# sj-shoff/ImageProcessor

Hardware: AMD Instinct MI355X
Metric: images/sec (resize+thumb+watermark) on 1080p batch at 1/2/4/8 MI355X (higher is better)
Workload: dtype f32+f64

## Files before the change

imageprocessor_amd/csrc/ipx_device.h:

```cpp
#pragma once

#include "ipx_internal.h"

namespace ipx {
namespace {

constexpr uint32_t kM = 0xffffu;

template <int C>
__device__ __forceinline__ double widen(uint32_t px)
{
    constexpr uint32_t sel = 0x0c0c0000u | (uint32_t)C | ((uint32_t)C << 8);
    return (double)__builtin_amdgcn_perm(0u, px, sel);
}

template <int C>
__device__ __forceinline__ uint32_t lerp_channel(uint32_t p00, uint32_t p10, uint32_t p01,
                                                 uint32_t p11, double xw0, double xw1, double yw0,
                                                 double yw1)
{
    const double s00 = widen<C>(p00), s10 = widen<C>(p10);
    const double s01 = widen<C>(p01), s11 = widen<C>(p11);
    const double top = xw0 * s00 + xw1 * s10;
    const double bot = xw0 * s01 + xw1 * s11;
// ... 1 lines not shown
    return (uint32_t)v;
}

__device__ __forceinline__ uint32_t pack_src(uint32_t pr, uint32_t pg, uint32_t pb, uint32_t pa)
{
    return (pr >> 8) | (pg & 0xff00u) | ((pb & 0xff00u) << 8) | ((pa & 0xff00u) << 16);
}

__device__ __forceinline__ uint32_t blend_over(uint32_t d, uint32_t pr, uint32_t pg, uint32_t pb,
                                               uint32_t pa)
{
    const uint32_t pa1 = (kM - pa) * 0x101u;
    const uint32_t r = (((d & 0xffu) * pa1 / kM + pr) >> 8) & 0xffu;
    const uint32_t g = ((((d >> 8) & 0xffu) * pa1 / kM + pg) >> 8) & 0xffu;
    const uint32_t b = ((((d >> 16) & 0xffu) * pa1 / kM + pb) >> 8) & 0xffu;
    const uint32_t a = (((d >> 24) * pa1 / kM + pa) >> 8) & 0xffu;
    return r | (g << 8) | (b << 16) | (a << 24);
}

__device__ __forceinline__ uint32_t glyph_over(uint32_t d, uint32_t mask8, uint32_t sr, uint32_t sg,
                                               uint32_t sb, uint32_t sa)
{
    const uint32_t ma = mask8 | (mask8 << 8);
    const uint32_t a = (kM - (sa * ma / kM)) * 0x101u;
    const uint32_t r = (((d & 0xffu) * a + sr * ma) / kM >> 8) & 0xffu;
    const uint32_t g = ((((d >> 8) & 0xffu) * a + sg * ma) / kM >> 8) & 0xffu;
    const uint32_t b = ((((d >> 16) & 0xffu) * a + sb * ma) / kM >> 8) & 0xffu;
    const uint32_t al = (((d >> 24) * a + sa * ma) / kM >> 8) & 0xffu;
    return r | (g << 8) | (b << 16) | (al << 24);
}

__device__ __forceinline__ uint32_t glyph_run(uint32_t d, int x, int y, const DevGlyph *__restrict__ gl,
                                              int n, uint32_t sr, uint32_t sg, uint32_t sb,
                                              uint32_t sa)
{
    for (int g = 0; g < n; g++) {
        const DevGlyph G = gl[g];
        if (x >= G.x0 && x < G.x1 && y >= G.y0 && y < G.y1) {
            const uint32_t m = G.mask[(size_t)(y - G.y0) * G.mstride + (x - G.x0)];
            if (m) d = glyph_over(d, m, sr, sg, sb, sa);
        }
    }
    return d;
}

template <int PX, int ROWS, int YSTEP>
__device__ __forceinline__ void glyph_walk(const DevGlyph *tab, int n, int x, int ybase, Rect bbox, uint32_t (&d)[ROWS][PX], uint32_t sr,
                                           uint32_t sg, uint32_t sb, uint32_t sa)
{
    static_assert(PX >= 1 && PX <= 4, "a row's mask bytes travel in one dword");
    for (int g = 0; g < n; g += 4) {
        uint32_t m[4][ROWS];
        bool any = false;
#pragma unroll
        for (int j = 0; j < 4; j++) {
            const DevGlyph G = tab[min(g + j, n - 1)];
#pragma unroll
            for (int r = 0; r < ROWS; r++) {
                const int y = ybase + YSTEP * r;
                const bool iny = g + j < n && y >= G.y0 && y < G.y1 && y < bbox.y1;
                uint32_t mm = 0u;
#pragma unroll
                for (int k = 0; k < PX; k++) {
                    const bool in = iny && x + k >= G.x0 && x + k < G.x1;
                    mm |= (in ? (uint32_t)G.mask[(size_t)(y - G.y0) * G.mstride + (x + k - G.x0)] : 0u) << (8 * k);
                    any |= in;
                }
                m[j][r] = mm;
            }
        }
        if (!__any(any)) continue;
#pragma unroll
        for (int j = 0; j < 4; j++)
#pragma unroll
            for (int r = 0; r < ROWS; r++)
#pragma unroll
                for (int k = 0; k < PX; k++) {
                    const uint32_t mk = (m[j][r] >> (8 * k)) & 0xffu;
                    if (mk) d[r][k] = glyph_over(d[r][k], mk, sr, sg, sb, sa);
                }
    }
}

}
}
```

imageprocessor_amd/csrc/ipx_internal.h:

```cpp
#pragma once

#include <hip/hip_runtime.h>

#include <cstdarg>
#include <cstdint>
#include <cstdio>
#include <map>
#include <mutex>

#include "../../include/ipx.h"

namespace ipx {

void set_error(const char *fmt, ...) __attribute__((format(printf, 1, 2)));
void clear_error();
int status_of_exception() noexcept;
#define IPX_CATCH_STATUS catch (...) { return ipx::status_of_exception(); }

#define IPX_HIP(call)                                                                        \
    do {                                                                                     \
        hipError_t e_ = (call);                                                              \
        if (e_ != hipSuccess) {                                                              \
            ipx::set_error("%s failed: %s (%s:%d)", #call, hipGetErrorString(e_), __FILE__,  \
                           __LINE__);                                                        \
            return IPX_ERR_HIP;                                                              \
        }                                                                                    \
    } while (0)

constexpr long long kMaxFrameSpan = 0x7fff0000LL;
constexpr int kMaxFrameSide = 65535;
inline bool frame_span_ok(long long w, long long h, long long stride, int bpp)
{
    if (w > kMaxFrameSide || h > kMaxFrameSide) return false;
    return w <= 0 || h <= 0 || (h - 1) * stride + w * bpp <= kMaxFrameSpan;
}

struct Rect {
    int x0, y0, x1, y1;
    int dx() const { return x1 - x0; }
    int dy() const { return y1 - y0; }
    bool empty() const { return x0 >= x1 || y0 >= y1; }
    Rect shifted(int ox, int oy) const { return Rect{x0 + ox, y0 + oy, x1 + ox, y1 + oy}; }
    Rect intersect(const Rect &s) const;
};
inline Rect to_rect(const ipx_rect &r) { return Rect{r.x0, r.y0, r.x1, r.y1}; }

bool draw_clip(Rect &r, int dw, int dh, bool has_src, int sw, int sh, int &spx, int &spy,
               bool has_mask, int mw, int mh, int &mpx, int &mpy);

enum SrcType { kSrcRGBA, kSrcNRGBA, kSrcGray, kSrcPaletted, kSrcYCbCr, kSrcNRGBA64, kSrcRGBA64, kSrcGray16, kSrcCMYK, kSrcTypes };
inline int src_bpp(int type) { static const int b[kSrcTypes] = {4, 4, 1, 1, 1, 8, 8, 2, 4}; return b[type]; }
inline int src_of_deep(int k) { return k >= IPX_DEEP_NRGBA64 && k <= IPX_DEEP_CMYK ? kSrcNRGBA64 + k : -1; }
inline int src_of_png(int k)
{
    static const int t[] = {kSrcGray, kSrcNRGBA, kSrcRGBA, kSrcPaletted, kSrcGray16, kSrcRGBA64, kSrcNRGBA64};
    return k >= 0 && k < 7 ? t[k] : -1;
}
inline int src_of_job(int k)
{
    static const int t[] = {kSrcRGBA, -1, kSrcNRGBA, kSrcGray, kSrcNRGBA64, kSrcRGBA64, kSrcGray16, kSrcCMYK};
    return k >= 0 && k < 8 ? t[k] : -1;
}
inline void chroma_size(int ratio, int w, int h, int *cw, int *ch)
{
    *cw = ratio == IPX_YCBCR_422 || ratio == IPX_YCBCR_420 ? (w + 1) / 2 : w;
    *ch = ratio == IPX_YCBCR_420 || ratio == IPX_YCBCR_440 ? (h + 1) / 2 : h;
}

enum { IPX_SRC_RGBA = 0, IPX_SRC_NRGBA = 1, IPX_SRC_YCBCR = 2,
       IPX_SRC_TAP64 = 3  };
hipError_t launch_opaque_scan(const uint8_t *src, int sw, int sh, int sstride, int *flag,
                              hipStream_t s);
hipError_t launch_opaque_scan_tap64(const uint8_t *src, int sw, int sh, int sstride, int *flag, hipStream_t s);
hipError_t launch_draw(uint8_t *dst, int dstride, const uint8_t *src, int sstride, int w, int h,
                       int op, hipStream_t s);
hipError_t launch_draw_nrgba(uint8_t *dst, int dstride, const uint8_t *src, int sstride, int w, int h, int op,
                             hipStream_t s, int nframes = 1, size_t dst_fs = 0, size_t src_fs = 0);
hipError_t launch_deep_expand(uint8_t *dst, size_t dst_fs, const uint8_t *src, int sstride, size_t src_fs, int kind, int w, int h, int nframes, hipStream_t s);
hipError_t launch_draw_tap64(uint8_t *dst, int dstride, const uint8_t *src, int sstride, int w, int h, int op, hipStream_t s,
                             int nframes = 1, size_t dst_fs = 0, size_t src_fs = 0);
hipError_t launch_draw_ycbcr(uint8_t *dst, int dstride, const uint8_t *y, int ystride, const uint8_t *cb,
                             const uint8_t *cr, int cstride, int ratio, int spx, int spy, int w, int h, hipStream_t s,
                             int nframes = 1, size_t dst_fs = 0, size_t y_fs = 0, size_t c_fs = 0);

struct DevGlyph {
    const uint8_t *mask;
    int mstride;
    int x0, y0, x1, y1;
};
constexpr int kMaxGlyphs = 256;
hipError_t launch_stream_copy(void *dst, const void *src, size_t bytes, hipStream_t s);
hipError_t launch_composite(uint8_t *dst, int dstride, size_t frame_stride, int nframes,
                            const DevGlyph *glyphs_dev, int n, Rect bbox, uint32_t sr, uint32_t sg,
                            uint32_t sb, uint32_t sa, hipStream_t s);

hipError_t launch_gray_expand(uint8_t *dst, size_t dst_fs, const uint8_t *src, int sstride, size_t src_fs, int w, int h, int n, hipStream_t s);
hipError_t launch_palette_expand(uint8_t *dst, size_t dst_fs, const uint8_t *src, int sstride, size_t src_fs, const uint8_t *palettes, int w,
                                 int h, int n, hipStream_t s);

struct KernelLaunchCache {
    std::mutex mu;
    size_t lds_max = 0;
    std::map<size_t, int> resident;
    bool said = false;
    hipError_t prepare(const void *fn, int threads, size_t lds, int *res)
    {
        std::lock_guard<std::mutex> lk(mu);
        if (lds > lds_max) {
            hipError_t e = hipFuncSetAttribute(fn, hipFuncAttributeMaxDynamicSharedMemorySize, (int)lds);
            if (e != hipSuccess) return e;
            lds_max = lds;
        }
        if (res) {
            auto it = resident.find(lds);
            if (it == resident.end()) {
                int n = 0;
                hipError_t e = hipOccupancyMaxActiveBlocksPerMultiprocessor(&n, fn, threads, lds);
                if (e != hipSuccess) return e;
                it = resident.emplace(lds, n > 1 ? n : 1).first;
            }
            *res = it->second;
        }
        return hipSuccess;
    }
    bool first_report() { std::lock_guard<std::mutex> lk(mu); const bool f = !said; said = true; return f; }
};


struct JpegTables {
    uint8_t quant[2][64];
    uint16_t div8[2][64];
    uint32_t recip[2][64];
};
void jpeg_tables(int quality, JpegTables *t);
struct JpegArgs {
    const uint8_t *src; size_t frame_stride; int stride, w, h;
    int aligned16;
    int16_t *coefs; int mcus_per_frame;
    const uint32_t *huff;
    uint32_t *aclen;
    int16_t *dcq;
    uint32_t recip[2][64];
    uint16_t div8[2][64];
};
hipError_t launch_jpeg_fdct(const JpegArgs &a, int n, hipStream_t s);


struct JpegDecInfo {
    int w, h, h0, v0, ratio, ri, ncomp;
    int host_scans;
    int progressive;
    uint8_t td[3], ta[3];
    size_t scan_off, scan_len;
};
struct JpegDecTables {
    uint16_t lut[4][256];
    int32_t maxcode[4][18];
    int32_t valoff[4][18];
    uint8_t vals[4][256];
    uint16_t qnat[3][64];
    uint32_t bound[4][8];
};
struct JpegDecImage {
    unsigned long long scan_off; uint32_t scan_len, img, first_mcu, n_mcu;
    uint8_t td[3], ta[3], valid, pad;
    uint8_t strict_end, rsv[3];
    unsigned long long uoff;
    uint32_t tab_img, rsv2;
};
struct JpegDecArgs {
    const uint8_t *blob; const JpegDecImage *img; const JpegDecTables *tab;
    int16_t *coefs; int *status;
    int16_t *dcs;
// ... 67 lines not shown
```

imageprocessor_amd/csrc/ipx_ks.h:

```cpp
#pragma once

#include <vector>

#include "ipx_internal.h"

namespace ipx {

struct KsAxis {
    int dw = 0, sw = 0;
    int ntap = 0;
    std::vector<int32_t> lo, cnt;
    std::vector<double> w;
    std::vector<double> itw, itwffff;
    std::vector<double> ones;
};
bool ks_build_axis(int dw, int sw, KsAxis *out);

struct KsAxisDev {
    const int32_t *lo, *cnt;
    const double *w, *itw, *itwffff, *ones;
    int ntap;
};
size_t ks_axis_bytes(const KsAxis &a);
void ks_axis_pack(const KsAxis &a, uint8_t *h, const uint8_t *d, KsAxisDev *out);

enum {
    IPX_SRC_RGBA_CROP = 8,
    IPX_SRC_NRGBA_CROP = 9,
    IPX_SRC_YCBCR_CROP = 10,
    IPX_SRC_TAP64_CROP = 11
};
inline int ks_crop_kind(int kind)
{
    return kind == IPX_SRC_NRGBA ? IPX_SRC_NRGBA_CROP : kind == IPX_SRC_YCBCR ? IPX_SRC_YCBCR_CROP : kind == IPX_SRC_TAP64 ? IPX_SRC_TAP64_CROP
                                                                                                                           : IPX_SRC_RGBA_CROP;
}

struct KsGenArgs {
    uint8_t *dst; int dstride; size_t dst_fs;
    int dr_x0, dr_y0;
    int adr_x0, adr_y0, adr_x1, adr_y1;
    int sr_x0, sr_y0;
    KsAxisDev ax, ay;
    int op;
    const int *opaque_flag;
    int kind;
    const uint8_t *src; int sstride; size_t src_fs;
    const uint8_t *cb, *cr; int cstride, ratio; size_t c_fs;
    int nframes;
    int src_w;
};
hipError_t launch_ks_generic(const KsGenArgs &a, hipStream_t s);

}

namespace ipx {

struct KsStrip { int c0, c1, t0, tw; };
struct KsSeg { int ys, r0, r1; };
template <int NACC> struct KsRowT { double w[NACC], itw[NACC], ones[NACC]; int32_t emit[NACC]; float wf[NACC]; };
static_assert(sizeof(KsRowT<2>) == 64 && sizeof(KsRowT<4>) == 128, "row entries are copied dword-wise");

struct KsFusedOut {
    uint8_t *out; size_t frame_stride; int ostride, obytes;
    int dw, dh, sr_x0, sr_y0;
    int kind;
    int mode, aone;
    int pk;
    int ntap;
    int waves, cpl;
    int wcols;
    const double *wx;
    const float *wxf;
    int split, ntapf;
    float feps;
    const double *itwf;
    const int32_t *xlo;
    const int32_t *colb;
    const void *rows;
    const int32_t *rowoff;
};
struct KsFusedArgs {
    const uint8_t *src; size_t src_fs; int sstride, sw, sh;
    int src_kind;
    int taps_le_alpha;
    const uint8_t *cb, *cr; int cstride, ratio; size_t c_fs;
    uint8_t *wm; size_t wm_fs; int wm_stride;
    int nframes, nstrips, nseg, nthreads, pitch, dbuf;
    const KsStrip *strips; const KsSeg *segs;
    int nout; KsFusedOut o[2];
    int lds_w[2], lds_rows, lds_open;
    int open_per_wave;
    uint8_t wave_role[16];
    unsigned long long *stamps;
    int *redo;
    uint2 *fix; int *fix_count; int fix_cap[2], fix_stride;
};
struct KsText { const DevGlyph *gl; int n; Rect bbox; uint32_t sr, sg, sb, sa; };
struct KsFix { uint2 *list = nullptr; int *count = nullptr; int cap[2] = {0, 0}; KsAxisDev ax[2], ay[2]; };
struct KsFusedGeom { int nseg = 0; const KsSeg *segs = nullptr; const void *rows[2] = {nullptr, nullptr}; const int32_t *rowoff[2] = {nullptr, nullptr}; };
struct KsFusedPlan {
    bool ok = false;
    int nacc = 2, rows = 4, pitch = 0, nstrips = 0, nthreads = 0, nstg = 0, dbuf = 0;
    int lds_w[2] = {0, 0}, lds_rows = 0, lds_open = 0, lds_bytes = 0;
    struct Lds { int dbuf = 0, lds_w[2] = {0, 0}, lds_rows = 0, lds_open = 0, open_per_wave = 0, lds_bytes = 0; } fast;
    const KsStrip *strips = nullptr;
    struct Out { int ntap = 0, waves = 0, cpl = 0, wcols = 0; const double *wx = nullptr, *itwf = nullptr; const int32_t *xlo = nullptr, *colb = nullptr;
                 const float *wxf = nullptr; float feps = 0; int split = 1, ntapf = 0; } o[2];
    KsFusedGeom whole, split;
};
constexpr int kKsSplitRows = 96;
constexpr int kKsRows = 4;
constexpr int kKsMaxStage = 3;
constexpr int kKsMaxWaves = 12;
constexpr int kKsMaxThreads = 64 * kKsMaxWaves;
constexpr int kKsMaxCpl = 2;
constexpr int kKsSplitTaps = 16;
constexpr int kKsOpenPerWave = 128;
struct KsFusedIn { int dw, dh, sr_x0, sr_y0; const KsAxis *hx, *hy; int top_taps = 0; };
bool ks_fused_plan(int sw, int sh, const KsFusedIn *sc0, const KsFusedIn *sc1, int px_bytes, std::vector<uint8_t> *blob, KsFusedPlan *out);
void ks_fused_rebase(KsFusedPlan *p, const uint8_t *dev_blob);
hipError_t launch_ks_fused(const KsFusedPlan &p, KsFusedArgs &a, const KsFix *fix, const KsText *text, int cus, hipStream_t s, bool *matched, bool *text_done);
hipError_t launch_ks_fix(const KsGenArgs &g, const uint2 *list, size_t list_stride, const int *count, int count_stride, int cap, hipStream_t s);

struct KsTailArgs {
    KsGenArgs g[2];
    const uint2 *list[2]; const int *count[2]; int cap[2];
    size_t list_stride; int count_stride;
    int nframes;
    int R[2], chunks[2];
    uint8_t *wm; int wm_stride; size_t wm_fs;
    KsText text;
    int tbx, tby;
};
hipError_t launch_ks_tail(KsTailArgs t, hipStream_t s);

}
```

imageprocessor_amd/csrc/ipx_ks_tail.hip:

```cpp
#include <algorithm>
#include <cstdlib>

#include "ipx_ks_exact.h"

namespace ipx {
namespace {

constexpr int kTailThreads = 256;
constexpr int kTextRows = 4;

template <int KIND>
__device__ __forceinline__ void tail_exact(KsGenArgs a, const uint2 *list, size_t list_stride, const int *count, int count_stride, int cap, int R,
                                           int frame, int chunk, int chunks)
{
    const int n = min(count[(size_t)frame * count_stride], cap);
    list += (size_t)frame * list_stride;
    a.dst += frame * a.dst_fs;
    a.src += frame * a.src_fs;
    if (KIND == IPX_SRC_YCBCR || KIND == IPX_SRC_YCBCR_CROP) { a.cb += frame * a.c_fs; a.cr += frame * a.c_fs; }
    const int lane = (int)threadIdx.x & 63, wv = (int)threadIdx.x >> 6;
    const int per_wave = 64 / R, sub = lane / R, sl = lane - sub * R, per_block = (kTailThreads >> 6) * per_wave;
    ks_exact_list<KIND>(a, list, n, chunk * per_block, chunks * per_block, wv * per_wave + sub, R, sub, sl);
}

__device__ __forceinline__ void tail_text(const KsTailArgs &t, DevGlyph *tab, int f, int rb)
{
    const int by = rb / t.tbx, bx = rb - by * t.tbx;
    const Rect bbox = t.text.bbox;
    const int n = t.text.n;
    const int x = bbox.x0 + bx * 64 + ((int)threadIdx.x & 63);
    const int ybase = bbox.y0 + by * (4 * kTextRows) + ((int)threadIdx.x >> 6);
    uint8_t *frame = t.wm + (size_t)f * t.wm_fs;
    uint32_t d[kTextRows][1], d0[kTextRows];
#pragma unroll
    for (int r = 0; r < kTextRows; r++) {
        const int y = ybase + 4 * r;
        d0[r] = d[r][0] = x < bbox.x1 && y < bbox.y1 ? *(const uint32_t *)(frame + (size_t)y * t.wm_stride + (size_t)x * 4) : 0u;
    }
    for (int g = (int)threadIdx.x; g < n; g += kTailThreads) tab[g] = t.text.gl[g];
    __syncthreads();
    glyph_walk<1, kTextRows, 4>(tab, n, x, ybase, bbox, d, t.text.sr, t.text.sg, t.text.sb, t.text.sa);
#pragma unroll
    for (int r = 0; r < kTextRows; r++) {
        const int y = ybase + 4 * r;
        if (x < bbox.x1 && y < bbox.y1 && d[r][0] != d0[r]) *(uint32_t *)(frame + (size_t)y * t.wm_stride + (size_t)x * 4) = d[r][0];
    }
}

template <int K0, int K1>
__global__ __launch_bounds__(kTailThreads) void ks_tail_kernel(KsTailArgs t)
{
    __shared__ DevGlyph tab[kMaxGlyphs];
    const int nx = t.chunks[0] + t.chunks[1], per = nx + t.tbx * t.tby, b = (int)blockIdx.x;
    const int frame = b / per, c = b - frame * per;
    if (c < nx) {
        const int k = c >= t.chunks[0] ? 1 : 0, chunk = c - (k ? t.chunks[0] : 0);
        if (K0 == K1 || k == 0)
            tail_exact<K0>(k ? t.g[1] : t.g[0], t.list[k], t.list_stride, t.count[k], t.count_stride, t.cap[k], t.R[k], frame, chunk, t.chunks[k]);
        else
            tail_exact<K1>(t.g[1], t.list[1], t.list_stride, t.count[1], t.count_stride, t.cap[1], t.R[1], frame, chunk, t.chunks[1]);
        return;
    }
    tail_text(t, tab, frame, c - nx);
}

template <int K0, int K1>
void tail_go(const KsTailArgs &t, unsigned blocks, hipStream_t s)
{
    hipLaunchKernelGGL((ks_tail_kernel<K0, K1>), dim3(blocks), dim3(kTailThreads), 0, s, t);
}

template <int S, int C>
bool tail_pair(int k0, int k1, const KsTailArgs &t, unsigned blocks, hipStream_t s)
{
    if (k0 == S && k1 == S) tail_go<S, S>(t, blocks, s);
    else if (k0 == S && k1 == C) tail_go<S, C>(t, blocks, s);
    else if (k0 == C && k1 == C) tail_go<C, C>(t, blocks, s);
    else return false;
    return true;
}

}

hipError_t launch_ks_tail(KsTailArgs t, hipStream_t s)
{
    if (t.nframes <= 0) return hipSuccess;
    const char *ev = getenv("IPX_KS_TAIL_BLOCKS");
    const int budget = ev && atoi(ev) > 0 ? atoi(ev) : 2048;
    for (int k = 0; k < 2; k++) {
        t.R[k] = 8; t.chunks[k] = 0;
        if (!t.list[k] || t.cap[k] <= 0) { t.cap[k] = 0; continue; }
        const int ntap = t.g[k].ay.ntap;
        t.R[k] = ntap <= 4 ? 4 : ntap <= 8 ? 8 : ntap <= 16 ? 16 : 64;
        const int per_block = (kTailThreads / 64) * (64 / t.R[k]), most = (t.cap[k] + per_block - 1) / per_block;
        t.chunks[k] = std::max(1, std::min(most, std::max(1, budget / t.nframes)));
    }
    const bool text = t.wm && t.text.gl && t.text.n > 0 && !t.text.bbox.empty();
    if (!text) t.text.n = 0;
    t.tbx = text ? (t.text.bbox.dx() + 63) / 64 : 0;
    t.tby = text ? (t.text.bbox.dy() + 4 * kTextRows - 1) / (4 * kTextRows) : 0;
    const long long blocks = (long long)t.nframes * (t.chunks[0] + t.chunks[1]) + (long long)t.nframes * t.tbx * t.tby;
    if (blocks <= 0) return hipSuccess;
    if (blocks > 0x7fffffffLL) return hipErrorInvalidValue;
    const int k0 = t.chunks[0] ? t.g[0].kind : t.g[1].kind, k1 = t.chunks[1] ? t.g[1].kind : k0;
    const bool none = !t.chunks[0] && !t.chunks[1];
    if (none) { tail_go<IPX_SRC_RGBA, IPX_SRC_RGBA>(t, (unsigned)blocks, s); return hipGetLastError(); }
    if (!tail_pair<IPX_SRC_RGBA, IPX_SRC_RGBA_CROP>(k0, k1, t, (unsigned)blocks, s) && !tail_pair<IPX_SRC_NRGBA, IPX_SRC_NRGBA_CROP>(k0, k1, t, (unsigned)blocks, s) &&
        !tail_pair<IPX_SRC_YCBCR, IPX_SRC_YCBCR_CROP>(k0, k1, t, (unsigned)blocks, s) && !tail_pair<IPX_SRC_TAP64, IPX_SRC_TAP64_CROP>(k0, k1, t, (unsigned)blocks, s))
        return hipErrorInvalidValue;
    return hipGetLastError();
}

}
```

imageprocessor_amd/csrc/ipx_runtime.hip:

```cpp
#include <algorithm>
#include <chrono>
#include <condition_variable>
#include <cstdlib>
#include <cstring>
#include <map>
#include <mutex>
#include <new>
#include <thread>
#include <utility>
#include <vector>

#include "ipx_runtime_internal.h"
#include "ipx_ks.h"

#ifndef IPX_DIAG
#define IPX_DIAG 0
#endif

namespace {

struct ScalePrep {
    bool empty;
    Rect adr;
};
// ... 67 lines not shown
    else if (src.kind == IPX_SRC_TAP64)
        IPX_HIP(launch_draw_tap64(d, dstride, src.pix + (size_t)spy * src.stride + (size_t)spx * 8, src.stride, r.dx(), r.dy(), op, s,
                                  src.nframes, dst_fs, src.frame_stride));
    else
        for (int i = 0; i < std::max(1, src.nframes); i++)
            IPX_HIP(launch_draw(d + (size_t)i * dst_fs, dstride, src.pix + (size_t)i * src.frame_stride + (size_t)spy * src.stride + (size_t)spx * 4,
                                src.stride, r.dx(), r.dy(), op, s));
    return IPX_OK;
}

int dev_scale_src(ipx_ctx *ctx, hipStream_t s, int *flag, uint8_t *dst, int dw, int dh, int dstride, const Rect &dr,
                  const DevSrc &src, const Rect &sr, int op, size_t dst_fs = 0, int kind_override = -1, const KsAxisDev *axes = nullptr)
{
    ScalePrep pr;
    int rc = scale_prepare(dw, dh, dr, src.w, src.h, sr, op, &pr);
    if (rc) return rc;
    if (pr.empty) return IPX_OK;
    if (src.kind == IPX_SRC_YCBCR) op = IPX_OP_SRC;
    if (op == IPX_OP_OVER && src.kind == IPX_SRC_TAP64) IPX_HIP(launch_opaque_scan_tap64(src.pix, src.w, src.h, src.stride, flag, s));
    else if (op == IPX_OP_OVER) IPX_HIP(launch_opaque_scan(src.pix, src.w, src.h, src.stride, flag, s));
    KsGenArgs a{};
    if (axes) { a.ax = axes[0]; a.ay = axes[1]; }
    else {
        if ((rc = ks_axis_get(ctx, dr.dx(), sr.dx(), &a.ax))) return rc;
        if ((rc = ks_axis_get(ctx, dr.dy(), sr.dy(), &a.ay))) return rc;
    }
    a.dst = dst; a.dstride = dstride; a.src = src.pix; a.sstride = src.stride;
    a.dr_x0 = dr.x0; a.dr_y0 = dr.y0;
    a.adr_x0 = pr.adr.x0; a.adr_y0 = pr.adr.y0; a.adr_x1 = pr.adr.x1; a.adr_y1 = pr.adr.y1;
    a.sr_x0 = sr.x0; a.sr_y0 = sr.y0;
    a.op = op; a.opaque_flag = op == IPX_OP_OVER ? flag : nullptr;
    a.kind = kind_override >= 0 ? kind_override : src.kind;
    a.cb = src.cb; a.cr = src.cr; a.cstride = src.cstride; a.ratio = src.ratio;
    a.nframes = src.nframes; a.src_fs = src.frame_stride; a.c_fs = src.c_frame_stride; a.dst_fs = dst_fs;
    IPX_HIP(launch_ks_generic(a, s));
    return IPX_OK;
}

DevSrc rgba_src(const uint8_t *p, int w, int h, int stride, int kind = IPX_SRC_RGBA)
{
    DevSrc d;
    d.kind = kind; d.pix = p; d.stride = stride; d.w = w; d.h = h;
    return d;
}

int dev_draw(hipStream_t s, uint8_t *dst, int dw, int dh, int dstride, Rect r, const uint8_t *src,
             int sw, int sh, int sstride, int spx, int spy, int op)
{
    return dev_draw_src(s, dst, dw, dh, dstride, r, rgba_src(src, sw, sh, sstride), spx, spy, op);
}

int dev_scale(ipx_ctx *ctx, hipStream_t s, int *flag, uint8_t *dst, int dw, int dh, int dstride, const Rect &dr,
              const uint8_t *src, int sw, int sh, int sstride, const Rect &sr, int op)
{
    return dev_scale_src(ctx, s, flag, dst, dw, dh, dstride, dr, rgba_src(src, sw, sh, sstride), sr, op);
}

int glyphs_for_frame(const ipx_glyphset *gs, int dw, int dh, ClippedGlyphs *out)
{
    std::lock_guard<std::mutex> lk(gs->mu);
    auto it = gs->clipped.find({dw, dh});
    if (it != gs->clipped.end()) { *out = it->second; return IPX_OK; }
    std::vector<DevGlyph> tab;
    Rect bb{0, 0, 0, 0};
    for (const GlyphHost &g : gs->g) {
        Rect r = g.dr;
        int spx = 0, spy = 0, mpx = g.mpx, mpy = g.mpy;
        if (!draw_clip(r, dw, dh, false, 0, 0, spx, spy, true, g.mw, g.mh, mpx, mpy)) continue;
        DevGlyph d;
        d.mask = gs->masks_dev + g.mask_off + (size_t)mpy * g.mw + mpx;
        d.mstride = g.mw;
        d.x0 = r.x0; d.y0 = r.y0; d.x1 = r.x1; d.y1 = r.y1;
        if (tab.empty()) bb = r;
        else {
            bb.x0 = std::min(bb.x0, r.x0); bb.y0 = std::min(bb.y0, r.y0);
            bb.x1 = std::max(bb.x1, r.x1); bb.y1 = std::max(bb.y1, r.y1);
        }
        tab.push_back(d);
    }
    ClippedGlyphs c;
    c.n = (int)tab.size();
    c.bbox = bb;
    if (c.n) {
        IPX_HIP(hipMalloc((void **)&c.dev, tab.size() * sizeof(DevGlyph)));
        IPX_HIP(hipMemcpy(c.dev, tab.data(), tab.size() * sizeof(DevGlyph), hipMemcpyHostToDevice));
    }
    gs->clipped[{dw, dh}] = c;
    *out = c;
    return IPX_OK;
}

int dev_composite(hipStream_t s, uint8_t *dst, int dw, int dh, int dstride, size_t frame_stride,
                  int nframes, const ipx_glyphset *gs)
{
    ClippedGlyphs c;
    int rc = glyphs_for_frame(gs, dw, dh, &c);
    if (rc) return rc;
    IPX_HIP(launch_composite(dst, dstride, frame_stride, nframes, c.dev, c.n, c.bbox,
                             gs->col[0] * 0x101u, gs->col[1] * 0x101u, gs->col[2] * 0x101u,
                             gs->col[3] * 0x101u, s));
    return IPX_OK;
}

}

extern "C" {

static void prepare_hip_env();
int ipx_device_count(void) try
{
    prepare_hip_env();
    clear_error();
    int n = 0;
    hipError_t e = hipGetDeviceCount(&n);
    if (e != hipSuccess) { (void)hipGetLastError(); set_error("hipGetDeviceCount: %s", hipGetErrorString(e)); return IPX_ERR_NODEVICE; }
    return n;
}
IPX_CATCH_STATUS

static void prepare_hip_env()
{
    static std::once_flag once;
    std::call_once(once, [] {
        if (!getenv("GPU_MAX_HW_QUEUES")) {
            char v[16];
            snprintf(v, sizeof v, "%d", std::max(8, env_int("IPX_LANES", 5) + 3));
            setenv("GPU_MAX_HW_QUEUES", v, 0);
        }
    });
}

int ipx_create(const ipx_config *cfg, ipx_ctx **out) try
{
    clear_error();
    if (!out) { set_error("ipx_create: null out"); return IPX_ERR_INVALID; }
    *out = nullptr;
    prepare_hip_env();
    int ndev = 0;
    if (hipGetDeviceCount(&ndev) != hipSuccess || ndev <= 0) {
        (void)hipGetLastError();
        set_error("no HIP device visible: the pixel path has no CPU fallback");
        return IPX_ERR_NODEVICE;
    }
    int dev = cfg ? cfg->device : -1;
    if (dev < 0) dev = env_int("IPX_DEVICE", env_int("LOCAL_RANK", 0) % ndev);
    if (dev >= ndev) { set_error("device %d out of range (%d visible)", dev, ndev); return IPX_ERR_INVALID; }
    IPX_HIP(hipSetDevice(dev));
    hipDeviceProp_t prop;
    IPX_HIP(hipGetDeviceProperties(&prop, dev));
    if (strncmp(prop.gcnArchName, "gfx950", 6) != 0) {
        set_error("device %d is %s; libipx carries gfx950 code only", dev, prop.gcnArchName);
        return IPX_ERR_NODEVICE;
    }
    ipx_ctx *c = new (std::nothrow) ipx_ctx;
    if (!c) { set_error("out of memory"); return IPX_ERR_NOMEM; }
    c->device = dev;
    c->cus = prop.multiProcessorCount > 0 ? prop.multiProcessorCount : 256;
    int lanes = cfg && cfg->lanes > 0 ? cfg->lanes : env_int("IPX_LANES", 5);
    c->lane_bytes = cfg && cfg->lane_bytes ? cfg->lane_bytes : (size_t)64 << 20;
    c->host_cache_limit = (size_t)std::max(0, env_int("IPX_HOST_CACHE_MB", 8192)) << 20;
    c->lanes.resize(lanes);
    int prio_lo = 0, prio_hi = 0;
    (void)hipDeviceGetStreamPriorityRange(&prio_lo, &prio_hi);
    hipError_t e = hipSuccess;
    if (c->lanes.size() >= 3) e = hipStreamCreateWithPriority(&c->lanes.back().stream, hipStreamNonBlocking, prio_hi);
    if (e == hipSuccess) e = hipStreamCreateWithFlags(&c->stream, hipStreamNonBlocking);
    for (size_t i = 0; i < c->lanes.size(); i++) {
        Lane &l = c->lanes[i];
// ... 841 lines not shown
int ipx_plan_query(const ipx_plan *plan, ipx_plan_info *info) try
{
    clear_error();
    if (!plan || !info) { set_error("ipx_plan_query: bad argument"); return IPX_ERR_INVALID; }
    *info = plan->info;
    return IPX_OK;
}
IPX_CATCH_STATUS

}

static hipError_t composite_text(const ipx_plan *pl, uint8_t *wm, size_t wm_frame_stride, int n, hipStream_t s)
{
    if (!wm || pl->glyphs.n <= 0 || !pl->p.glyphs) return hipSuccess;
    const uint8_t *c = pl->p.glyphs->col;
    return launch_composite(wm, pl->p.sw * 4, wm_frame_stride, n, pl->glyphs.dev, pl->glyphs.n, pl->glyphs.bbox, c[0] * 0x101u, c[1] * 0x101u,
                            c[2] * 0x101u, c[3] * 0x101u, s);
}

static int run_dev_any(ipx_ctx *ctx, hipStream_t s, const ipx_plan *pl, int n, const DevSrc &src, uint8_t *resize_out, size_t resize_frame_stride,
                       uint8_t *thumb_out, size_t thumb_frame_stride, uint8_t *wm_out, size_t wm_frame_stride)
{
    const int sw = pl->p.sw, sh = pl->p.sh;
    uint8_t *outs[2] = {pl->sc[0].on ? resize_out : nullptr, pl->sc[1].on ? thumb_out : nullptr};
    const size_t ostr[2] = {resize_frame_stride, thumb_frame_stride};
    uint8_t *wm = pl->p.do_watermark ? wm_out : nullptr;
    for (int k = 0; k < 2; k++)
        if (pl->sc[k].dw <= 0 || pl->sc[k].dh <= 0) outs[k] = nullptr;
    if (!wm && !outs[0] && !outs[1]) return IPX_OK;
    int kinds[2] = {src.kind, pl->p.crop_to_fit ? ks_crop_kind(src.kind) : src.kind};

    const bool gray = src.kind == IPX_SRC_YCBCR && src.cstride == 0;
    const KsFusedPlan &fp = pl->fused[src.kind == IPX_SRC_RGBA ? 0 : gray ? 2 : 1];
    if (fp.ok && env_int("IPX_FUSED", 1)) {
        KsFusedArgs a{};
        a.src = src.pix; a.src_fs = src.frame_stride; a.sstride = src.stride; a.sw = sw; a.sh = sh;
        a.src_kind = src.kind; a.cb = src.cb; a.cr = src.cr; a.cstride = src.cstride; a.ratio = src.ratio; a.c_fs = src.c_frame_stride;
        a.wm = wm; a.wm_fs = wm_frame_stride; a.wm_stride = sw * 4;
        a.nframes = n;
        a.taps_le_alpha = src.le_alpha;
        for (int k = 0; k < 2; k++) {
            if (!outs[k]) continue;
            const PlanScale &ps = pl->sc[k];
            KsFusedOut &o = a.o[a.nout++];
            o.out = outs[k]; o.frame_stride = ostr[k]; o.ostride = ps.dw * 4; o.obytes = ps.dw * ps.dh * 4;
            o.dw = ps.dw; o.dh = ps.dh; o.sr_x0 = ps.sr.x0; o.sr_y0 = ps.sr.y0;
            o.kind = kinds[k]; o.pk = k;
        }
        AsyncFree mem{s, {}};
        int *redo = nullptr;
        KsFix fixv, *fix = nullptr;
        const int max_items = n * fp.nstrips * std::max(fp.whole.nseg, fp.split.nseg);
        const bool spec = src.kind == IPX_SRC_RGBA && env_int("IPX_KS_SPEC", 1);
        const bool fast = (spec || src.kind == IPX_SRC_YCBCR || src.kind == IPX_SRC_NRGBA || (src.kind == IPX_SRC_TAP64 && src.le_alpha)) &&
                          env_int("IPX_KS_FAST", 1) != 0;
        if (spec || fast) {
            const int cap_env = env_int("IPX_KS_FIX_CAP", 0);
            int cap[2] = {0, 0};
            for (int k = 0; k < 2; k++)
                if (fast && outs[k]) cap[k] = cap_env > 0 ? cap_env : (int)std::min<size_t>(std::max<size_t>((size_t)pl->sc[k].dw * pl->sc[k].dh / 96, 256), (size_t)1 << 20);
            const size_t flags = align256((size_t)max_items * sizeof(int)), counts = fast ? align256((size_t)n * 2 * sizeof(int)) : 0;
            IPX_HIP(mem.get(&redo, flags + counts + (size_t)n * (cap[0] + cap[1]) * sizeof(uint2)));
            if (fast) {
                fixv.count = (int *)((uint8_t *)redo + flags);
                fixv.list = (uint2 *)((uint8_t *)redo + flags + counts);
                fixv.cap[0] = cap[0]; fixv.cap[1] = cap[1];
                for (int k = 0; k < 2; k++) { fixv.ax[k] = pl->sc[k].ax[0]; fixv.ay[k] = pl->sc[k].ax[1]; }
                IPX_HIP(hipMemsetAsync(fixv.count, 0, (size_t)n * 2 * sizeof(int), s));
                fix = &fixv;
            }
        }
        a.redo = redo;
#if IPX_DIAG
        static unsigned long long *stamp_buf = nullptr;
        if (env_int("IPX_STAMPS", 0)) {
            if (!stamp_buf) IPX_HIP(hipMalloc((void **)&stamp_buf, 24 * sizeof(unsigned long long)));
            IPX_HIP(hipMemsetAsync(stamp_buf, 0, 24 * sizeof(unsigned long long), s));
            a.stamps = stamp_buf;
        }
#endif
        KsText text{}, *txt = nullptr;
        if (wm && pl->glyphs.n > 0 && pl->p.glyphs) {
            const uint8_t *c = pl->p.glyphs->col;
            text = KsText{pl->glyphs.dev, pl->glyphs.n, pl->glyphs.bbox, c[0] * 0x101u, c[1] * 0x101u, c[2] * 0x101u, c[3] * 0x101u};
            txt = &text;
        }
        bool matched = false, text_done = false;
        hipError_t e = launch_ks_fused(fp, a, fix, txt, ctx->cus, s, &matched, &text_done);
        if (fix && matched && e == hipSuccess && env_int("IPX_KS_STATS", 0)) {
            std::vector<int> cnt((size_t)n * 2), flags((size_t)max_items);
            (void)hipMemcpyAsync(cnt.data(), fixv.count, cnt.size() * sizeof(int), hipMemcpyDeviceToHost, s);
            (void)hipMemcpyAsync(flags.data(), redo, flags.size() * sizeof(int), hipMemcpyDeviceToHost, s);
            (void)hipStreamSynchronize(s);
            long long tot[2] = {0, 0}; int mx[2] = {0, 0}, nredo = 0;
            for (int i = 0; i < n; i++) for (int k = 0; k < 2; k++) { tot[k] += cnt[2 * i + k]; mx[k] = std::max(mx[k], cnt[2 * i + k]); }
            for (int f : flags) nredo += f != 0;
            fprintf(stderr, "[ipx ks stats] %d frames: undecided pixels per frame resize mean %.1f max %d (room %d), thumbnail mean %.1f max %d (room %d); %d of %d items redone in float64\n", n,
                    (double)tot[0] / n, mx[0], fixv.cap[0], (double)tot[1] / n, mx[1], fixv.cap[1], nredo, max_items);
        }
#if IPX_DIAG
        if (a.stamps && matched) {
            unsigned long long h[24];
            IPX_HIP(hipMemcpyAsync(h, a.stamps, sizeof h, hipMemcpyDeviceToHost, s));
            IPX_HIP(hipStreamSynchronize(s));
            const char *who[3] = {"resize waves", "thumbnail waves", "idle waves"};
            for (int r = 0; r < 3; r++) {
                double tot = 0;
                for (int i = 0; i < 6; i++) tot += (double)h[r * 8 + i];
                if (tot > 0)
                    fprintf(stderr, "[ipx stamps] %-16s share of wave time: wait-loads %.1f%%  drain %.1f%%  barrier %.1f%%  issue %.1f%%  scaleX %.1f%%  scaleY %.1f%%  (%.3g cycles)\n", who[r],
                            100 * h[r * 8] / tot, 100 * h[r * 8 + 1] / tot, 100 * h[r * 8 + 2] / tot, 100 * h[r * 8 + 3] / tot, 100 * h[r * 8 + 4] / tot, 100 * h[r * 8 + 5] / tot, tot);
            }
        }
#endif
        if (e != hipSuccess) { set_error("one-pass kernel launch failed: %s", hipGetErrorString(e)); return IPX_ERR_HIP; }
        if (matched) {
            if (!text_done) IPX_HIP(composite_text(pl, wm, wm_frame_stride, n, s));
            return IPX_OK;
        }
    }

    if (wm) {
        const int rc = dev_draw_src(s, wm, sw, sh, sw * 4, Rect{0, 0, sw, sh}, src, 0, 0, IPX_OP_SRC, wm_frame_stride);
        if (rc) return rc;
        IPX_HIP(composite_text(pl, wm, wm_frame_stride, n, s));
    }
    for (int k = 0; k < 2; k++) {
        if (!outs[k]) continue;
        const PlanScale &ps = pl->sc[k];
        const int rc = dev_scale_src(ctx, s, nullptr, outs[k], ps.dw, ps.dh, ps.dw * 4, Rect{0, 0, ps.dw, ps.dh}, src, ps.sr, IPX_OP_SRC, ostr[k],
                                     kinds[k], ps.ax);
        if (rc) return rc;
    }
    return IPX_OK;
}


int src_check(const char *who, const ipx_plan *pl, const BatchSrc &b, int n, bool in_hbm)
{
    if (b.type < 0 || b.type >= kSrcTypes) { set_error("%s: unknown source type", who); return IPX_ERR_INVALID; }
    const int bpp = src_bpp(b.type);
    bool ok = pl && n >= 0 && b.plane[0] && (long long)b.stride[0] >= (long long)pl->p.sw * bpp;
    if (ok && b.type == kSrcYCbCr) {
        int cw = 0, ch = 0;
        chroma_size(b.ratio, pl->p.sw, pl->p.sh, &cw, &ch);
        ok = b.plane[1] && b.plane[2] && b.ratio >= 0 && b.ratio <= IPX_YCBCR_440 && b.stride[1] >= cw;
    }
    if (ok && b.type == kSrcPaletted) ok = b.palettes && !(in_hbm && ((uintptr_t)b.palettes & 3));
    if (ok && in_hbm && b.type >= kSrcNRGBA64)
        ok = !(((uintptr_t)b.plane[0] | (uintptr_t)b.stride[0] | b.frame_stride[0]) & (b.type == kSrcCMYK ? 3 : 1));
    if (!ok) { set_error("%s: bad argument", who); return IPX_ERR_INVALID; }
    const int sw = pl->p.sw, sh = pl->p.sh;
    if (!frame_span_ok(sw, sh, b.stride[0], bpp) || (b.type == kSrcYCbCr && !frame_span_ok(sw, sh, b.stride[1], 1)) ||
        (b.type >= kSrcNRGBA64 && !frame_span_ok(sw, sh, (long long)sw * 8, 8))) {
        set_error("%s: %dx%d frames with row strides of %d / %d bytes are beyond the 2 GiB span the kernels address", who, sw, sh, b.stride[0], b.stride[1]);
        return IPX_ERR_UNSUPPORTED;
    }
    if (in_hbm && n > 65535) { set_error("%s: at most 65535 frames per call", who); return IPX_ERR_UNSUPPORTED; }
    return IPX_OK;
}

SrcLayout src_layout(const ipx_plan *pl, const BatchSrc &b, size_t (*frame_rule)(size_t))
{
    SrcLayout L{};
    int cw = 0, ch = 0;
    if (b.type == kSrcYCbCr) chroma_size(b.ratio, pl->p.sw, pl->p.sh, &cw, &ch);
    L.planes = b.type == kSrcYCbCr ? 3 : 1;
// ... 395 lines not shown
```

imageprocessor_amd/csrc/ipx_runtime_internal.h:

```cpp
#pragma once

#include <sched.h>

#include <algorithm>
#include <cctype>
#include <cstdio>
#include <condition_variable>
#include <cstdlib>
#include <cstring>
#include <deque>
#include <map>
#include <mutex>
#include <string>
#include <utility>
#include <vector>

#include "ipx_internal.h"
#include "ipx_ks.h"

using namespace ipx;

struct Lane {
    hipStream_t stream = nullptr;
    uint8_t *dev = nullptr;
    size_t dev_bytes = 0;
    int *flag = nullptr;
    uint8_t *dec = nullptr;
    size_t dec_bytes = 0;
    uint8_t *pin = nullptr;
    size_t pin_bytes = 0;
    hipEvent_t ev[3] = {nullptr, nullptr, nullptr};
    bool busy = false;
};

struct ipx_ctx {
    int device = 0;
    int cus = 256;
    hipStream_t stream = nullptr;
    std::vector<Lane> lanes;
    size_t lane_bytes = 0;
    std::mutex mu;
    std::condition_variable cv;
    std::mutex host_mu;
    std::map<void *, size_t> host_size;
    std::multimap<size_t, void *> host_free_blocks;
    std::deque<void *> host_lru;
    size_t host_cached = 0, host_cache_limit = (size_t)8 << 30;
    int jj_active = 0;
    uint8_t *flat_chroma = nullptr;
    std::mutex plan_mu;
    std::map<std::string, std::pair<ipx_glyphset *, ipx_plan *>> plan_cache;
    uint64_t plan_clock = 0;
    std::mutex ks_mu;
    std::map<std::pair<int, int>, std::pair<uint8_t *, KsAxisDev>> ks_axes;
    static constexpr size_t kFlatChromaBytes = (size_t)64 << 10;
};

struct GlyphHost {
    size_t mask_off;
    int mw, mh;
    Rect dr;
    int mpx, mpy;
};

struct ClippedGlyphs {
    DevGlyph *dev = nullptr;
    int n = 0;
    Rect bbox{0, 0, 0, 0};
};

struct ipx_glyphset {
    int device = 0;
    std::vector<GlyphHost> g;
    uint8_t *masks_dev = nullptr;
    size_t masks_bytes = 0;
    uint8_t col[4] = {0, 0, 0, 0};
    mutable std::mutex mu;
    mutable std::map<std::pair<int, int>, ClippedGlyphs> clipped;
};

struct PlanScale {
    bool on = false;
    int dw = 0, dh = 0;
    Rect sr{0, 0, 0, 0};
    KsAxis hx, hy;
    KsAxisDev ax[2]{};
};

struct ipx_plan {
    ipx_plan_params p{};
    ipx_plan_info info{};
    PlanScale sc[2];
    KsFusedPlan fused[3];
    uint8_t *blob = nullptr;
    ClippedGlyphs glyphs;
    mutable std::mutex mu;
    ipx_glyphset *owned_gs = nullptr;
    int cache_refs = 0;
    uint64_t cache_stamp = 0;
};

inline int env_int(const char *name, int dflt)
{
    const char *v = getenv(name);
    return v && *v ? atoi(v) : dflt;
}

struct DeviceGuard {
    explicit DeviceGuard(int dev) { ok = hipSetDevice(dev) == hipSuccess; }
    bool ok;
};

#define IPX_ENTER(ctx)                                                         \
    clear_error();                                                             \
    if (!(ctx)) { set_error("%s: null context", __func__); return IPX_ERR_INVALID; } \
    DeviceGuard guard_((ctx)->device);                                         \
    if (!guard_.ok) { set_error("hipSetDevice(%d) failed", (ctx)->device); return IPX_ERR_HIP; }

class LaneLease {
public:
    explicit LaneLease(ipx_ctx *c) : c_(c)
    {
        std::unique_lock<std::mutex> lk(c->mu);
        c->cv.wait(lk, [&] {
            for (auto &l : c->lanes) if (!l.busy) return true;
            return false;
        });
        for (auto &l : c->lanes) if (!l.busy) { l.busy = true; lane_ = &l; break; }
    }
    ~LaneLease()
    {
        {
            std::lock_guard<std::mutex> lk(c_->mu);
            lane_->busy = false;
        }
        c_->cv.notify_all();
    }
    Lane *operator->() { return lane_; }
    Lane &get() { return *lane_; }
private:
    ipx_ctx *c_;
    Lane *lane_ = nullptr;
};

inline int lane_reserve_dec(Lane &l, size_t bytes)
{
    if (bytes <= l.dec_bytes) return IPX_OK;
    if (l.dec) { IPX_HIP(hipStreamSynchronize(l.stream)); IPX_HIP(hipFree(l.dec)); l.dec = nullptr; l.dec_bytes = 0; }
    const size_t want = bytes + bytes / 8;
    hipError_t e = hipMalloc((void **)&l.dec, want);
    if (e != hipSuccess) {
// ... 195 lines not shown
```

Baseline: 252,500.

## Index glyphs per column so tail text blocks walk only covering glyphs

Builds a per-column glyph index on the host when glyphs are clipped. Columns are split into single-glyph and multi-glyph lists. The text tail kernel now maps each thread to a column that is actually covered, instead of to every x in the bounding box. Each thread walks only the glyphs that cover its column, rather than scanning all glyphs in groups of four, which cuts idle threads and wasted glyph tests. The cost is extra host setup and device memory, plus an indirect column load per thread.

```diff
diff --git a/imageprocessor_amd/csrc/ipx_device.h b/imageprocessor_amd/csrc/ipx_device.h
--- a/imageprocessor_amd/csrc/ipx_device.h
+++ b/imageprocessor_amd/csrc/ipx_device.h
@@ -107,5 +107,26 @@
     }
 }
 
+template <int ROWS, int YSTEP>
+__device__ __forceinline__ void glyph_walk_cols(const DevGlyph *tab, const uint8_t *idx, int cnt, int x, int ybase, int y1, uint32_t (&d)[ROWS],
+                                                uint32_t sr, uint32_t sg, uint32_t sb, uint32_t sa)
+{
+    uint32_t gi = cnt > 0 ? idx[0] : 0u;
+    for (int k = 0; k < cnt; k++) {
+        const DevGlyph G = tab[gi];
+        if (k + 1 < cnt) gi = idx[k + 1];
+        uint32_t m[ROWS];
+#pragma unroll
+        for (int r = 0; r < ROWS; r++) {
+            const int y = ybase + YSTEP * r;
+            const bool in = y >= G.y0 && y < G.y1 && y < y1;
+            m[r] = in ? (uint32_t)G.mask[(size_t)(y - G.y0) * G.mstride + (x - G.x0)] : 0u;
+        }
+#pragma unroll
+        for (int r = 0; r < ROWS; r++)
+            if (m[r]) d[r] = glyph_over(d[r], m[r], sr, sg, sb, sa);
+    }
+}
+
 }
 }
diff --git a/imageprocessor_amd/csrc/ipx_internal.h b/imageprocessor_amd/csrc/ipx_internal.h
--- a/imageprocessor_amd/csrc/ipx_internal.h
+++ b/imageprocessor_amd/csrc/ipx_internal.h
@@ -89,6 +89,8 @@
     int x0, y0, x1, y1;
 };
 constexpr int kMaxGlyphs = 256;
+struct GlyphCol { int x, first, cnt; };
+struct GlyphCols { const uint8_t *idx; const GlyphCol *list[2]; int n[2]; };
 hipError_t launch_stream_copy(void *dst, const void *src, size_t bytes, hipStream_t s);
 hipError_t launch_composite(uint8_t *dst, int dstride, size_t frame_stride, int nframes,
                             const DevGlyph *glyphs_dev, int n, Rect bbox, uint32_t sr, uint32_t sg,
diff --git a/imageprocessor_amd/csrc/ipx_ks.h b/imageprocessor_amd/csrc/ipx_ks.h
--- a/imageprocessor_amd/csrc/ipx_ks.h
+++ b/imageprocessor_amd/csrc/ipx_ks.h
@@ -96,7 +96,7 @@
     int *redo;
     uint2 *fix; int *fix_count; int fix_cap[2], fix_stride;
 };
-struct KsText { const DevGlyph *gl; int n; Rect bbox; uint32_t sr, sg, sb, sa; };
+struct KsText { const DevGlyph *gl; int n; Rect bbox; uint32_t sr, sg, sb, sa; GlyphCols cols; };
 struct KsFix { uint2 *list = nullptr; int *count = nullptr; int cap[2] = {0, 0}; KsAxisDev ax[2], ay[2]; };
 struct KsFusedGeom { int nseg = 0; const KsSeg *segs = nullptr; const void *rows[2] = {nullptr, nullptr}; const int32_t *rowoff[2] = {nullptr, nullptr}; };
 struct KsFusedPlan {
@@ -131,7 +131,7 @@
     int R[2], chunks[2];
     uint8_t *wm; int wm_stride; size_t wm_fs;
     KsText text;
-    int tbx, tby;
+    int tbx, tby, tc0;
 };
 hipError_t launch_ks_tail(KsTailArgs t, hipStream_t s);
 
diff --git a/imageprocessor_amd/csrc/ipx_ks_tail.hip b/imageprocessor_amd/csrc/ipx_ks_tail.hip
--- a/imageprocessor_amd/csrc/ipx_ks_tail.hip
+++ b/imageprocessor_amd/csrc/ipx_ks_tail.hip
@@ -28,22 +28,25 @@
     const int by = rb / t.tbx, bx = rb - by * t.tbx;
     const Rect bbox = t.text.bbox;
     const int n = t.text.n;
-    const int x = bbox.x0 + bx * 64 + ((int)threadIdx.x & 63);
+    const int li = bx >= t.tc0 ? 1 : 0, ci = (bx - (li ? t.tc0 : 0)) * 64 + ((int)threadIdx.x & 63);
+    const bool has = ci < t.text.cols.n[li];
+    const GlyphCol col = has ? t.text.cols.list[li][ci] : GlyphCol{0, 0, 0};
+    const int x = col.x;
     const int ybase = bbox.y0 + by * (4 * kTextRows) + ((int)threadIdx.x >> 6);
     uint8_t *frame = t.wm + (size_t)f * t.wm_fs;
-    uint32_t d[kTextRows][1], d0[kTextRows];
+    uint32_t d[kTextRows], d0[kTextRows];
 #pragma unroll
     for (int r = 0; r < kTextRows; r++) {
         const int y = ybase + 4 * r;
-        d0[r] = d[r][0] = x < bbox.x1 && y < bbox.y1 ? *(const uint32_t *)(frame + (size_t)y * t.wm_stride + (size_t)x * 4) : 0u;
+        d0[r] = d[r] = has && y < bbox.y1 ? *(const uint32_t *)(frame + (size_t)y * t.wm_stride + (size_t)x * 4) : 0u;
     }
     for (int g = (int)threadIdx.x; g < n; g += kTailThreads) tab[g] = t.text.gl[g];
     __syncthreads();
-    glyph_walk<1, kTextRows, 4>(tab, n, x, ybase, bbox, d, t.text.sr, t.text.sg, t.text.sb, t.text.sa);
+    glyph_walk_cols<kTextRows, 4>(tab, t.text.cols.idx + col.first, col.cnt, x, ybase, bbox.y1, d, t.text.sr, t.text.sg, t.text.sb, t.text.sa);
 #pragma unroll
     for (int r = 0; r < kTextRows; r++) {
         const int y = ybase + 4 * r;
-        if (x < bbox.x1 && y < bbox.y1 && d[r][0] != d0[r]) *(uint32_t *)(frame + (size_t)y * t.wm_stride + (size_t)x * 4) = d[r][0];
+        if (has && y < bbox.y1 && d[r] != d0[r]) *(uint32_t *)(frame + (size_t)y * t.wm_stride + (size_t)x * 4) = d[r];
     }
 }
 
@@ -97,7 +100,9 @@
     }
     const bool text = t.wm && t.text.gl && t.text.n > 0 && !t.text.bbox.empty();
     if (!text) t.text.n = 0;
-    t.tbx = text ? (t.text.bbox.dx() + 63) / 64 : 0;
+    if (text && (t.text.cols.n[0] + t.text.cols.n[1] <= 0 || !t.text.cols.idx)) return hipErrorInvalidValue;
+    t.tc0 = text ? (t.text.cols.n[0] + 63) / 64 : 0;
+    t.tbx = text ? t.tc0 + (t.text.cols.n[1] + 63) / 64 : 0;
     t.tby = text ? (t.text.bbox.dy() + 4 * kTextRows - 1) / (4 * kTextRows) : 0;
     const long long blocks = (long long)t.nframes * (t.chunks[0] + t.chunks[1]) + (long long)t.nframes * t.tbx * t.tby;
     if (blocks <= 0) return hipSuccess;
diff --git a/imageprocessor_amd/csrc/ipx_runtime.hip b/imageprocessor_amd/csrc/ipx_runtime.hip
--- a/imageprocessor_amd/csrc/ipx_runtime.hip
+++ b/imageprocessor_amd/csrc/ipx_runtime.hip
@@ -173,8 +173,28 @@
     c.n = (int)tab.size();
     c.bbox = bb;
     if (c.n) {
-        IPX_HIP(hipMalloc((void **)&c.dev, tab.size() * sizeof(DevGlyph)));
-        IPX_HIP(hipMemcpy(c.dev, tab.data(), tab.size() * sizeof(DevGlyph), hipMemcpyHostToDevice));
+        std::vector<uint8_t> idx;
+        std::vector<GlyphCol> list[2];
+        for (int x = bb.x0; x < bb.x1; x++) {
+            const int first = (int)idx.size();
+            for (int g = 0; g < c.n; g++)
+                if (x >= tab[g].x0 && x < tab[g].x1) idx.push_back((uint8_t)g);
+            const int cnt = (int)idx.size() - first;
+            if (cnt) list[cnt > 1].push_back(GlyphCol{x, first, cnt});
+        }
+        const size_t tab_b = tab.size() * sizeof(DevGlyph), l0_b = list[0].size() * sizeof(GlyphCol), l1_b = list[1].size() * sizeof(GlyphCol);
+        std::vector<uint8_t> blob(tab_b + l0_b + l1_b + idx.size());
+        memcpy(blob.data(), tab.data(), tab_b);
+        if (l0_b) memcpy(blob.data() + tab_b, list[0].data(), l0_b);
+        if (l1_b) memcpy(blob.data() + tab_b + l0_b, list[1].data(), l1_b);
+        if (!idx.empty()) memcpy(blob.data() + tab_b + l0_b + l1_b, idx.data(), idx.size());
+        uint8_t *dev = nullptr;
+        IPX_HIP(hipMalloc((void **)&dev, blob.size()));
+        c.dev = (DevGlyph *)dev;
+        IPX_HIP(hipMemcpy(dev, blob.data(), blob.size(), hipMemcpyHostToDevice));
+        c.cols.list[0] = (const GlyphCol *)(dev + tab_b); c.cols.n[0] = (int)list[0].size();
+        c.cols.list[1] = (const GlyphCol *)(dev + tab_b + l0_b); c.cols.n[1] = (int)list[1].size();
+        c.cols.idx = dev + tab_b + l0_b + l1_b;
     }
     gs->clipped[{dw, dh}] = c;
     *out = c;
@@ -1182,7 +1202,7 @@
         KsText text{}, *txt = nullptr;
         if (wm && pl->glyphs.n > 0 && pl->p.glyphs) {
             const uint8_t *c = pl->p.glyphs->col;
-            text = KsText{pl->glyphs.dev, pl->glyphs.n, pl->glyphs.bbox, c[0] * 0x101u, c[1] * 0x101u, c[2] * 0x101u, c[3] * 0x101u};
+            text = KsText{pl->glyphs.dev, pl->glyphs.n, pl->glyphs.bbox, c[0] * 0x101u, c[1] * 0x101u, c[2] * 0x101u, c[3] * 0x101u, pl->glyphs.cols};
             txt = &text;
         }
         bool matched = false, text_done = false;
diff --git a/imageprocessor_amd/csrc/ipx_runtime_internal.h b/imageprocessor_amd/csrc/ipx_runtime_internal.h
--- a/imageprocessor_amd/csrc/ipx_runtime_internal.h
+++ b/imageprocessor_amd/csrc/ipx_runtime_internal.h
@@ -67,6 +67,7 @@
     DevGlyph *dev = nullptr;
     int n = 0;
     Rect bbox{0, 0, 0, 0};
+    GlyphCols cols{};
 };
 
 struct ipx_glyphset {
```

Result: no change. 256,200 (median of 2 runs) (+1.5%).
